# yondonfu/ai-rtc-agent

Hardware: NVIDIA H100
Metric: frames/sec at 512x512 SD-Turbo img2img (1-step, stream-batch 1) (higher is better)
Workload: dtype f16

## Files before the change

### ai-rtc-agent_b200/csrc/epilogue.cuh

```cuda
#pragma once
#include "igemm.cuh"
#include "ptx.cuh"
#include "wgmma.cuh"

namespace b2 {

__device__ __forceinline__ float gelu_erf(float x) {
    return 0.5f * x * (1.0f + erff(x * 0.70710678118654752440f));
}

__device__ __forceinline__ void store_half16(__half* dst, const float* v, int nv, bool vec_ok) {
    if (nv == 16 && vec_ok) {
        uint4 u[2];
        __half2* h = reinterpret_cast<__half2*>(u);
#pragma unroll
        for (int i = 0; i < 8; ++i) h[i] = __floats2half2_rn(v[2 * i], v[2 * i + 1]);
        reinterpret_cast<uint4*>(dst)[0] = u[0];
        reinterpret_cast<uint4*>(dst)[1] = u[1];
    } else {
#pragma unroll
        for (int i = 0; i < 16; ++i)
            if (i < nv) dst[i] = __float2half_rn(v[i]);
    }
}
// ... 97 lines not shown
struct EpiRow {
    long orow;
    int b;
    bool ok;
    float mu, rstd;
};

__device__ __forceinline__ void store_half2(__half* dst, float x0, float x1, bool two, bool vec_ok) {
    if (two && vec_ok) {
        *reinterpret_cast<__half2*>(dst) = __floats2half2_rn(x0, x1);
    } else {
        dst[0] = __float2half_rn(x0);
        if (two) dst[1] = __float2half_rn(x1);
    }
}

__device__ __forceinline__ void rowstat_quad(const IgEpilogue& e, const EpiRow& rw, float s1, float s2, int lane) {
    s1 += __shfl_xor_sync(0xffffffffu, s1, 1);
    s2 += __shfl_xor_sync(0xffffffffu, s2, 1);
    s1 += __shfl_xor_sync(0xffffffffu, s1, 2);
    s2 += __shfl_xor_sync(0xffffffffu, s2, 2);
    if ((lane & 3) == 0 && rw.ok) rowstat_add(e, rw.orow, s1, s2);
}

template <int BN>
__device__ __forceinline__ void epi_frag(const IgEpilogue& e, const float (&acc)[BN / 2], const EpiRow (&rw)[2], int ntile,
                                         bool ln_fma, int lane) {
    const int q2 = 2 * (lane & 3);
    const bool vec_out = (e.ldc & 1) == 0;
    if (e.flags & IG_GEGLU) {
        constexpr int HALF = BN / 2;
        const int pv0 = ntile * BN, oc0 = ntile * HALF;
#pragma unroll
        for (int j = 0; j < HALF / 8; ++j) {
            const int c = 8 * j + q2;
#pragma unroll
            for (int h = 0; h < 2; ++h) {
                if (!rw[h].ok) continue;
                float v[2];
#pragma unroll
                for (int u = 0; u < 2; ++u) {
                    float a = acc[4 * j + 2 * h + u], g = acc[4 * (j + HALF / 8) + 2 * h + u];
                    const int pv = pv0 + c + u, pg = pv0 + HALF + c + u;
                    if (ln_fma) {
                        const float nmr = -rw[h].mu * rw[h].rstd;
                        a = fmaf(rw[h].rstd, a, fmaf(nmr, e.colsum[pv], e.colbias ? e.colbias[pv] : 0.f));
                        g = fmaf(rw[h].rstd, g, fmaf(nmr, e.colsum[pg], e.colbias ? e.colbias[pg] : 0.f));
                    } else {
                        if (e.colsum) {
                            a = rw[h].rstd * (a - rw[h].mu * e.colsum[pv]);
                            g = rw[h].rstd * (g - rw[h].mu * e.colsum[pg]);
                        }
                        if (e.colbias) {
                            a += e.colbias[pv];
                            g += e.colbias[pg];
                        }
                    }
                    v[u] = a * gelu_erf(g);
                }
                store_half2(e.out + rw[h].orow * e.ldc + oc0 + c, v[0], v[1], true, vec_out);
            }
        }
        return;
    }
    float s1[2] = {0.f, 0.f}, s2[2] = {0.f, 0.f};
#pragma unroll
    for (int j = 0; j < BN / 8; ++j) {
        const int col = ntile * BN + 8 * j + q2;
        if (col >= e.n_valid) continue;
        const bool two = col + 1 < e.n_valid;
        const bool transposed = e.out2 && col >= e.col2;
#pragma unroll
        for (int h = 0; h < 2; ++h) {
            if (!rw[h].ok) continue;
            float x[2] = {acc[4 * j + 2 * h], acc[4 * j + 2 * h + 1]};
            const float* bp = e.colbias ? e.colbias + (long)rw[h].b * e.colbias_bstride + col : nullptr;
            if (ln_fma) {
                const float nmr = -rw[h].mu * rw[h].rstd;
#pragma unroll
                for (int u = 0; u < 2; ++u)
                    x[u] = fmaf(rw[h].rstd, x[u], fmaf(nmr, e.colsum[col + u], bp && (u == 0 || two) ? bp[u] : 0.f));
            } else {
                if (e.colsum) {
#pragma unroll
                    for (int u = 0; u < 2; ++u)
                        if (u == 0 || two) x[u] = rw[h].rstd * (x[u] - rw[h].mu * e.colsum[col + u]);
                }
                if (bp) {
                    x[0] += bp[0];
                    if (two) x[1] += bp[1];
                }
                if (e.acc_scale != 1.0f) {
                    x[0] *= e.acc_scale;
                    x[1] *= e.acc_scale;
                }
                if (e.res) {
                    const __half* rp = e.res + rw[h].orow * e.ldr + col;
                    if (two && (e.ldr & 1) == 0) {
                        const float2 f = __half22float2(*reinterpret_cast<const __half2*>(rp));
                        x[0] += e.res_scale * f.x;
                        x[1] += e.res_scale * f.y;
                    } else {
                        x[0] += e.res_scale * __half2float(rp[0]);
                        if (two) x[1] += e.res_scale * __half2float(rp[1]);
                    }
                }
                if (e.flags & IG_RELU) {
                    x[0] = fmaxf(x[0], 0.f);
                    x[1] = fmaxf(x[1], 0.f);
                }
            }
            if (transposed) {
                __half* tp = e.out2 + (long)(col - e.col2) * e.ld2 + rw[h].orow;
                tp[0] = __float2half_rn(x[0]);
                if (two) tp[e.ld2] = __float2half_rn(x[1]);
                continue;
            }
            if (e.rowstat_out && !ln_fma) {
                const float r0 = __half2float(__float2half_rn(x[0]));
                const float r1 = two ? __half2float(__float2half_rn(x[1])) : 0.f;
                s1[h] += r0 + r1;
                s2[h] += r0 * r0 + r1 * r1;
            }
            store_half2(e.out + rw[h].orow * e.ldc + col, x[0], x[1], two, vec_out);
        }
    }
    if (e.rowstat_out && !ln_fma) {
        rowstat_quad(e, rw[0], s1[0], s2[0], lane);
        rowstat_quad(e, rw[1], s1[1], s2[1], lane);
    }
}

template <int BN>
__device__ __forceinline__ void frag_to_smem(float* dst, const float (&acc)[BN / 2], int r0, int lane, int c0, int nc, bool colmajor) {
    const int q2 = 2 * (lane & 3);
#pragma unroll
    for (int j = 0; j < BN / 8; ++j) {
        const int c = 8 * j + q2 - c0;
        if (c < 0 || c >= nc) continue;
#pragma unroll
        for (int h = 0; h < 2; ++h) {
            const int r = r0 + 8 * h;
            if (colmajor) {
                dst[c * 128 + r] = acc[4 * j + 2 * h];
                dst[(c + 1) * 128 + r] = acc[4 * j + 2 * h + 1];
            } else {
                *reinterpret_cast<float2*>(dst + (((c >> 2) * 128 + r) << 2) + (c & 3)) =
                    make_float2(acc[4 * j + 2 * h], acc[4 * j + 2 * h + 1]);
            }
        }
    }
}

}
```

### ai-rtc-agent_b200/csrc/igemm.cu

```cuda
#include "igemm.cuh"

#include <cudaTypedefs.h>
#include <stdarg.h>
#include <stdio.h>
#include <stdlib.h>
#include <string.h>

#include "epilogue.cuh"
#include "launch.cuh"
#include "ptx.cuh"

namespace b2 {

#ifdef B2_TIMELINE
#define B2_TS(stmt) stmt
#else
#define B2_TS(stmt)
#endif

static thread_local char g_err[1024] = "";
const char* b2_last_error() { return g_err; }
void b2_set_error(const char* fmt, ...) {
    va_list ap;
    va_start(ap, fmt);
// ... 114 lines not shown
    const int cr = PAIR ? (int)(blockIdx.x & 1) : 0;
    const int mt_first = (int)blockIdx.x;
    const int mt_step = (int)gridDim.x;
    const int mt_guard = PAIR ? cr : 0;

    const int num_mtiles = p.tiles_w * p.tiles_h * p.tiles_n;
    const int ntile = blockIdx.y;
    const int kb_begin = blockIdx.z * p.kb_per_split;
    const int kb_end = min(p.total_kb, kb_begin + p.kb_per_split);
    [[maybe_unused]] unsigned long long* ts = p.dbg_ts ? p.dbg_ts + ((size_t)(blockIdx.z * gridDim.y + blockIdx.y) * gridDim.x + blockIdx.x) * 8 : nullptr;
    B2_TS(if (ts && threadIdx.x == 0) ts[0] = globaltimer_ns();)

    if (threadIdx.x == IG_CONS) {
        for (int s = 0; s < p.nseg; ++s) tma_prefetch_desc(&p.tmA[s]);
        tma_prefetch_desc(&p.tmB);
        for (int s = 0; s < p.num_stages; ++s) {
            mbar_init(&full_bar[s], 1);
            mbar_init(&empty_bar[s], (PAIR ? 2 : 1) * (IG_CONS / 32));
        }
        fence_mbar_init();
    }
    if (PAIR) {
        cluster_arrive_relaxed();
        cluster_wait();
    }
    __syncthreads();

    pdl_launch_dependents();
    pdl_wait();
    B2_TS(if (ts && threadIdx.x == 0) ts[1] = globaltimer_ns();)

    if (warp == IG_CONS / 32) {
        if (lane == 0) {
            [[maybe_unused]] const uint16_t pair_mask = PAIR ? (uint16_t)(3u << (cluster_ctarank() & ~1u)) : (uint16_t)0;
            int stage = 0;
            uint32_t phase = 0;
            for (int mt = mt_first; mt - mt_guard < num_mtiles; mt += mt_step) {
                const int w0 = (mt % p.tiles_w) * p.tw, h0 = ((mt / p.tiles_w) % p.tiles_h) * p.th;
                const int n0 = (mt / (p.tiles_w * p.tiles_h)) * p.tn;
                int seg = 0, base = 0;
                while (seg < p.nseg - 1 && kb_begin >= base + p.seg_ntap[seg] * p.seg_cblocks[seg]) {
                    base += p.seg_ntap[seg] * p.seg_cblocks[seg];
                    ++seg;
                }
                int tap = (kb_begin - base) / p.seg_cblocks[seg];
                int cb = (kb_begin - base) % p.seg_cblocks[seg];
                for (int kb = kb_begin; kb < kb_end; ++kb) {
                    mbar_wait(&empty_bar[stage], phase ^ 1);
#ifdef B2_BOUND_STUDY
                    if (p.dbg_mode == 1 && kb >= kb_begin + p.num_stages) {
                        mbar_arrive(&full_bar[stage]);
                        if (++stage == p.num_stages) { stage = 0; phase ^= 1; }
                        continue;
                    }
#endif
                    mbar_expect_tx(&full_bar[stage], p.a_bytes + p.b_bytes);
                    uint8_t* sa = smem + (size_t)stage * stage_bytes;
                    uint8_t* sb = sa + A_BYTES;
                    int dy = 0, dx = 0;
                    if (p.seg_ntap[seg] == 9) {
                        dy = tap / 3 - 1;
                        dx = tap % 3 - 1;
                    }
                    tma_load_4d(p.swap ? sb : sa, &p.tmA[seg], &full_bar[stage], p.seg_c0[seg] + cb * IG_BK,
                                w0 * p.stride + dx, h0 * p.stride + dy, n0);
                    if (PAIR)
                        tma_load_2d_mc(sb + cr * (BN / 2) * 128, &p.tmB, &full_bar[stage], kb * IG_BK, ntile * BN + cr * (BN / 2), pair_mask);
                    else
                        tma_load_2d(p.swap ? sa : sb, &p.tmB, &full_bar[stage], kb * IG_BK, ntile * (p.swap ? IG_BM : BN));
                    B2_TS(if (ts && mt == (int)blockIdx.x && kb == kb_begin) ts[2] = globaltimer_ns();)
                    if (++cb == p.seg_cblocks[seg]) {
                        cb = 0;
                        if (++tap == p.seg_ntap[seg]) {
                            tap = 0;
                            ++seg;
                        }
                    }
                    if (++stage == p.num_stages) {
                        stage = 0;
                        phase ^= 1;
                    }
                }
            }
        }
    } else {
        const int wg = warp >> 2;
        const int r0 = wg * 64 + (warp & 3) * 16 + (lane >> 2);
        [[maybe_unused]] const uint32_t peer_empty = PAIR ? dsmem_map(smem_u32(empty_bar), cluster_ctarank() ^ 1u) : 0u;
        const IgEpilogue& e = p.epi;
        const bool ln_fma = e.colsum && !p.swap && !(e.flags & IG_SPLITK) && (e.ldc & 7) == 0 && (e.n_valid & 15) == 0;
        const uint32_t smem_base = smem_u32(smem);
        auto release = [&](int s) {
            if (lane == 0) {
                mbar_arrive(&empty_bar[s]);
                if (PAIR) mbar_arrive_remote(peer_empty + (uint32_t)s * 8u);
            }
        };
        int stage = 0;
        uint32_t phase = 0;
        int it = 0;
        for (int mt = mt_first; mt - mt_guard < num_mtiles; mt += mt_step, ++it) {
            float acc[BN / 2];
#pragma unroll
            for (int i = 0; i < BN / 2; ++i) acc[i] = 0.f;
            int prev = -1;
            for (int kb = kb_begin; kb < kb_end; ++kb) {
                mbar_wait(&full_bar[stage], phase);
                B2_TS(if (ts && it == 0 && kb == kb_begin && threadIdx.x == 0) ts[3] = globaltimer_ns();)
                const uint32_t sa = smem_base + (uint32_t)stage * stage_bytes;
                const uint64_t da = make_kmajor_sw128_desc(sa + (uint32_t)wg * (64 * 128));
                const uint64_t db = make_kmajor_sw128_desc(sa + A_BYTES);
#ifdef B2_BOUND_STUDY
                if (p.dbg_mode != 2)
#endif
                {
                    wgmma_fence_regs(acc);
                    wgmma_fence();
#pragma unroll
                    for (int k = 0; k < 4; ++k) Wgmma<BN>::ss(acc, da + 2 * k, db + 2 * k, 1u);
                    wgmma_commit();
                    wgmma_wait<1>();
                    wgmma_fence_regs(acc);
                }
                if (prev >= 0) release(prev);
                prev = stage;
                if (++stage == p.num_stages) {
                    stage = 0;
                    phase ^= 1;
                }
            }
            wgmma_wait<0>();
            wgmma_fence_regs(acc);
            if (prev >= 0) release(prev);
            B2_TS(if (ts && it == 0 && threadIdx.x == 0) ts[4] = globaltimer_ns();)

            const int w0 = (mt % p.tiles_w) * p.tw, h0 = ((mt / p.tiles_w) % p.tiles_h) * p.th;
            const int n0 = (mt / (p.tiles_w * p.tiles_h)) * p.tn;
            if (p.swap || (e.flags & IG_SPLITK)) {
                float* stg = reinterpret_cast<float*>(smem);
                cons_bar_sync();
                if (e.flags & IG_SPLITK) {
                    frag_to_smem<BN>(stg, acc, r0, lane, 0, BN, false);
                } else {
                    for (int c = 0; c < BN; c += SWAP_CH) {
                        SwapPre pre;
                        swap_prefetch(p, pre, SWAP_CH, c, ntile, n0, h0, w0, threadIdx.x);
                        frag_to_smem<BN>(stg, acc, r0, lane, c, SWAP_CH, true);
                        cons_bar_sync();
                        swap_store_chunk(p, pre, stg, ntile, threadIdx.x);
                        cons_bar_sync();
                    }
                }
            } else {
                EpiRow rw[2];
#pragma unroll
                for (int h = 0; h < 2; ++h) {
                    const int r = r0 + 8 * h;
                    const int wi = r % p.tw, hi = (r / p.tw) % p.th, ni = r / (p.tw * p.th);
                    const int n = n0 + ni, hh = h0 + hi, ww = w0 + wi;
                    rw[h].ok = (ni < p.tn) && (n < p.Nb) && (hh < p.Ho) && (ww < p.Wo);
                    rw[h].orow = ((long)n * p.Ho + hh) * p.Wo + ww;
                    rw[h].b = n;
                    ln_row_stats(e, rw[h].orow, rw[h].ok, rw[h].mu, rw[h].rstd);
                }
                epi_frag<BN>(e, acc, rw, ntile, ln_fma, lane);
            }
            B2_TS(if (ts && it == 0 && threadIdx.x == 0) ts[5] = globaltimer_ns();)
        }
    }
    if (p.epi.flags & IG_SPLITK) {
        const int mt = blockIdx.x;
        const int w0 = (mt % p.tiles_w) * p.tw, h0 = ((mt / p.tiles_w) % p.tiles_h) * p.th;
        const int n0 = (mt / (p.tiles_w * p.tiles_h)) * p.tn;
        const int splits = (int)gridDim.z;
        const int rk_mul = PAIR ? 2 : 1, rk_add = cr;
        cluster_sync_all();
        B2_TS(if (ts && threadIdx.x == 0) ts[6] = globaltimer_ns();)
        if (warp < IG_CONS / 32 && p.swap) {
            const int rank = (int)cluster_ctarank();
            const int cols_per = BN / splits;
            const int ch = cols_per < SWAP_CH ? cols_per : SWAP_CH;
            const int t = threadIdx.x & (IG_BM - 1);
            const int half = threadIdx.x >> 7;
            const uint32_t stg_local = smem_u32(smem);
            float* T = reinterpret_cast<float*>(smem + (size_t)BN * IG_BM * 4);
            for (int c = rank * cols_per; c < (rank + 1) * cols_per; c += ch) {
                SwapPre pre;
                swap_prefetch(p, pre, ch, c, ntile, n0, h0, w0, threadIdx.x);
                if (ch >= 16) {
                    for (int g = 4 * half; g < (ch >> 2); g += 8) {
                        float acc[16];
                        const int cc = ((c >> 2) + g) >> 2;
                        switch (splits) {
                            case 2: splitk_sum16<2>(stg_local, cc, t, acc); break;
                            case 4: splitk_sum16<4>(stg_local, cc, t, acc); break;
                            default: splitk_sum16<8>(stg_local, cc, t, acc); break;
                        }
#pragma unroll
                        for (int i = 0; i < 16; ++i) T[(4 * g + i) * IG_BM + t] = acc[i];
                    }
                } else {
                    const int gg = half;
                    float4 v[8];
#pragma unroll
                    for (int sidx = 0; sidx < 8; ++sidx)
                        v[sidx] = dsmem_ld_f4(dsmem_map(stg_local, (uint32_t)sidx) + (uint32_t)((((c >> 2) + gg) * IG_BM + t) * 16));
                    float4 a = make_float4(0.f, 0.f, 0.f, 0.f);
#pragma unroll
                    for (int sidx = 0; sidx < 8; ++sidx) { a.x += v[sidx].x; a.y += v[sidx].y; a.z += v[sidx].z; a.w += v[sidx].w; }
                    T[(4 * gg + 0) * IG_BM + t] = a.x;
                    T[(4 * gg + 1) * IG_BM + t] = a.y;
                    T[(4 * gg + 2) * IG_BM + t] = a.z;
                    T[(4 * gg + 3) * IG_BM + t] = a.w;
                }
                cons_bar_sync();
                swap_store_chunk(p, pre, T, ntile, threadIdx.x);
                cons_bar_sync();
            }
        } else if (warp < IG_CONS / 32) {
            const int rank = (int)cluster_ctarank() / rk_mul;
            const int rows_per = IG_BM / splits;
            const int t = threadIdx.x;
            const int chunks = BN >> 4;
            const uint32_t stg_local = smem_u32(smem);
            for (int item = t; item < rows_per * chunks; item += IG_CONS) {
                const int rl = item % rows_per;
                const int cc = item / rows_per;
                const int r = rank * rows_per + rl;
                const int wi = r % p.tw, hi = (r / p.tw) % p.th, ni = r / (p.tw * p.th);
                const int n = n0 + ni, h = h0 + hi, w = w0 + wi;
                const bool ok = (ni < p.tn) && (n < p.Nb) && (h < p.Ho) && (w < p.Wo);
                float acc[16];
                switch (splits) {
                    case 2: splitk_sum16<2>(stg_local, cc, r, acc, rk_mul, rk_add); break;
                    case 4: splitk_sum16<4>(stg_local, cc, r, acc, rk_mul, rk_add); break;
                    default: splitk_sum16<8>(stg_local, cc, r, acc, rk_mul, rk_add); break;
                }
                if (ok) {
                    const long orow = ((long)n * p.Ho + h) * p.Wo + w;
                    float mu, rstd;
                    ln_row_stats(p.epi, orow, true, mu, rstd);
                    epi_store16<0>(p.epi, acc, n, orow, ntile * BN + cc * 16, mu, rstd);
                }
            }
        }
        B2_TS(if (ts && threadIdx.x == 0) ts[7] = globaltimer_ns();)
        cluster_sync_all();
    }
    if (PAIR) {
        cluster_arrive_relaxed();
        cluster_wait();
    }
}

template <int BN, bool PAIR>
__global__ void __launch_bounds__(IG_THREADS, 1) igemm_kernel(const __grid_constant__ IgemmParams p) { igemm_body<BN, PAIR>(p); }

using IgemmFn = void (*)(IgemmParams);
template <bool PAIR>
static IgemmFn igemm_fn(int bn) {
    switch (bn) {
#define B2_IG_CASE(N) case N: if constexpr (PAIR && (N % 32)) return nullptr; else return igemm_kernel<N, PAIR>;
        B2_IG_CASE(16) B2_IG_CASE(32) B2_IG_CASE(48) B2_IG_CASE(64) B2_IG_CASE(80) B2_IG_CASE(96) B2_IG_CASE(112) B2_IG_CASE(128)
        B2_IG_CASE(144) B2_IG_CASE(160) B2_IG_CASE(176) B2_IG_CASE(192) B2_IG_CASE(208) B2_IG_CASE(224) B2_IG_CASE(240) B2_IG_CASE(256)
#undef B2_IG_CASE
        default: return nullptr;
    }
}

static PFN_cuTensorMapEncodeTiled_v12000 get_encode() {
    static PFN_cuTensorMapEncodeTiled_v12000 fn = nullptr;
    if (fn) return fn;
    void* p = nullptr;
    cudaDriverEntryPointQueryResult qres;
    cudaError_t err = cudaGetDriverEntryPoint("cuTensorMapEncodeTiled", &p, cudaEnableDefault, &qres);
    if (err != cudaSuccess || qres != cudaDriverEntryPointSuccess || !p) {
        b2_set_error("cudaGetDriverEntryPoint(cuTensorMapEncodeTiled) failed: %s",
                     cudaGetErrorString(err));
        return nullptr;
    }
    fn = reinterpret_cast<PFN_cuTensorMapEncodeTiled_v12000>(p);
    return fn;
}

static thread_local bool g_plan_dry = false;
void igemm_set_dry_run(bool on) { g_plan_dry = on; }

static int encode_act_map(CUtensorMap* m, const ActView& a, int box_c, int box_w, int box_h, int box_n,
                          int estride) {
    if (g_plan_dry) return 0;
    auto enc = get_encode();
    if (!enc) return -1;
    cuuint64_t dims[4] = {(cuuint64_t)a.C, (cuuint64_t)a.W, (cuuint64_t)a.H, (cuuint64_t)a.N};
    cuuint64_t strides[3] = {(cuuint64_t)a.ld * 2, (cuuint64_t)a.W * a.ld * 2,
                             (cuuint64_t)a.H * a.W * a.ld * 2};
    cuuint32_t box[4] = {(cuuint32_t)box_c, (cuuint32_t)box_w, (cuuint32_t)box_h, (cuuint32_t)box_n};
    cuuint32_t es[4] = {1, (cuuint32_t)estride, (cuuint32_t)estride, 1};
    CUresult r = enc(m, CU_TENSOR_MAP_DATA_TYPE_FLOAT16, 4, const_cast<__half*>(a.ptr), dims, strides,
                     box, es, CU_TENSOR_MAP_INTERLEAVE_NONE, CU_TENSOR_MAP_SWIZZLE_128B,
                     CU_TENSOR_MAP_L2_PROMOTION_L2_256B, CU_TENSOR_MAP_FLOAT_OOB_FILL_NONE);
    if (r != CUDA_SUCCESS) {
        b2_set_error("cuTensorMapEncodeTiled(act) failed: %d (ptr %p dims %d,%d,%d,%d ld %d box "
                     "%d,%d,%d,%d es %d)",
                     (int)r, a.ptr, a.C, a.W, a.H, a.N, a.ld, box_c, box_w, box_h, box_n, estride);
        return -1;
    }
    return 0;
}

static int encode_w_map(CUtensorMap* m, const __half* w, int rows, int ld, int box_rows) {
    if (g_plan_dry) return 0;
    auto enc = get_encode();
    if (!enc) return -1;
    cuuint64_t dims[2] = {(cuuint64_t)ld, (cuuint64_t)rows};
    cuuint64_t strides[1] = {(cuuint64_t)ld * 2};
    cuuint32_t box[2] = {IG_BK, (cuuint32_t)box_rows};
    cuuint32_t es[2] = {1, 1};
    CUresult r = enc(m, CU_TENSOR_MAP_DATA_TYPE_FLOAT16, 2, const_cast<__half*>(w), dims, strides, box,
                     es, CU_TENSOR_MAP_INTERLEAVE_NONE, CU_TENSOR_MAP_SWIZZLE_128B,
                     CU_TENSOR_MAP_L2_PROMOTION_L2_256B, CU_TENSOR_MAP_FLOAT_OOB_FILL_NONE);
    if (r != CUDA_SUCCESS) {
        b2_set_error("cuTensorMapEncodeTiled(weights) failed: %d (rows %d ld %d box %d)", (int)r, rows,
                     ld, box_rows);
        return -1;
    }
    return 0;
}

size_t igemm_partial_floats(int splits, long rows_total, int n_valid) {
    long n_pad = ((n_valid + 255) / 256 + 1) * 256;
    return (size_t)splits * rows_total * n_pad;
}

static int plan_swap(const IgemmDesc& d, IgemmPlan* plan) {
    IgemmParams& p = plan->p;
    if ((d.epi.flags & IG_GEGLU) || d.nseg < 1 || d.nseg > IG_MAX_SRC || d.epi.rowstat_out || d.epi.colsum || d.epi.out2) {
        b2_set_error("igemm(swap): unsupported (GEGLU / LayerNorm fold / row statistics / transposed V / nseg %d)", d.nseg);
        return -1;
    }
    int BN = d.BN;
    const long rows_total = (long)d.Nb * d.Ho * d.Wo;
    if (BN <= 0) BN = rows_total >= 256 ? 256 : (rows_total >= 128 ? 128 : 64);
    if (BN != 64 && BN != 128 && BN != 256) {
        b2_set_error("igemm(swap): BN %d must be 64, 128 or 256", BN);
        return -1;
    }
    p.swap = 1;
    { static const char* dm = getenv("B2_DBG_MODE"); p.dbg_mode = dm ? atoi(dm) : 0; }
    p.acc_bufs = 1;
    p.BN = BN;
    auto lg = [](int v) { int l = 0; while ((1 << l) < v) ++l; return l; };
    int tw, th, tn;
    if (d.Ho == 1 && d.Nb == 1) { tw = BN; th = 1; tn = 1; }
    else if (d.Wo >= 16) { tw = 16; th = BN / 16; tn = 1; }
    else { tw = 8; th = 8; tn = BN / 64; }
    p.tw = tw; p.th = th; p.tn = tn;
    p.tw_log2 = lg(tw); p.th_log2 = lg(th);
    p.tiles_w = (d.Wo + tw - 1) / tw;
    p.tiles_h = (d.Ho + th - 1) / th;
    p.tiles_n = (d.Nb + tn - 1) / tn;
    p.Wo = d.Wo; p.Ho = d.Ho; p.Nb = d.Nb;
    p.stride = d.stride < 1 ? 1 : d.stride;
    p.nseg = d.nseg;
    int total_kb = 0;
    for (int s = 0; s < d.nseg; ++s) {
        const ActView& a = d.src[s];
        if (a.C % IG_BK != 0 || (a.ld % 8) != 0 || (reinterpret_cast<uintptr_t>(a.ptr) & 15) || (d.ntap[s] != 1 && d.ntap[s] != 9)) {
            b2_set_error("igemm(swap): bad source %d", s);
            return -1;
        }
        p.seg_ntap[s] = d.ntap[s];
        p.seg_cblocks[s] = a.C / IG_BK;
        p.seg_c0[s] = 0;
        total_kb += d.ntap[s] * p.seg_cblocks[s];
        if (encode_act_map(&p.tmA[s], a, IG_BK, tw * p.stride, th * p.stride, tn, p.stride)) return -1;
    }
    p.total_kb = total_kb;
    if (d.w_ld < total_kb * IG_BK || (d.w_ld % 8) != 0 || (reinterpret_cast<uintptr_t>(d.w) & 15)) {
        b2_set_error("igemm(swap): weight ld %d < K %d or misaligned", d.w_ld, total_kb * IG_BK);
        return -1;
    }
    if (encode_w_map(&p.tmB, d.w, d.w_rows, d.w_ld, IG_BM)) return -1;
    p.a_bytes = IG_BM * IG_BK * 2;
    p.b_bytes = (uint32_t)BN * IG_BK * 2;
    int splits = d.splits < 1 ? 1 : d.splits;
    if (splits > total_kb) splits = total_kb;
    if (splits >= 8) splits = 8; else if (splits >= 4) splits = 4; else if (splits >= 2) splits = 2;
    p.kb_per_split = (total_kb + splits - 1) / splits;
    while (splits > 1 && (total_kb + p.kb_per_split - 1) / p.kb_per_split != splits) {
        splits >>= 1;
        p.kb_per_split = (total_kb + splits - 1) / splits;
    }
    plan->splits = splits;
    plan->rows_total = rows_total;
    p.epi = d.epi;
    p.dbg_ts = d.dbg_ts;
    if (splits > 1) p.epi.flags |= IG_SPLITK;
    const int c_tiles = (d.epi.n_valid + IG_BM - 1) / IG_BM;
    p.n_pad = c_tiles * IG_BM;
    if ((d.epi.n_valid & 7) || (d.epi.ldc & 7) || (d.epi.res && (d.epi.ldr & 7)) || (d.epi.colbias && (d.epi.colbias_bstride & 3)) ||
        (reinterpret_cast<uintptr_t>(d.epi.out) & 15) || (reinterpret_cast<uintptr_t>(d.epi.res) & 15) ||
        (reinterpret_cast<uintptr_t>(d.epi.colbias) & 15)) {
        b2_set_error("igemm(swap): epilogue needs n_valid/ldc/ldr multiples of 8 and 16-byte aligned pointers");
        return -1;
    }
    const size_t stage_bytes = (size_t)IG_BM * IG_BK * 2 + (size_t)BN * IG_BK * 2;
    static const char* sw_stage_env = getenv("B2_SWAP_STAGE_KB");
    int stages = (int)(((size_t)(sw_stage_env ? atoi(sw_stage_env) : (d.ring_kb > 0 ? d.ring_kb : 200)) * 1024) / stage_bytes);
    if (stages < 2) stages = 2;
    if (stages > IG_MAX_STAGES) stages = IG_MAX_STAGES;
    if (stages > p.kb_per_split) stages = p.kb_per_split < 2 ? 2 : p.kb_per_split;
    size_t pipe_bytes = stages * stage_bytes;
    {
        const int cols_per = BN / splits;
        const size_t need = (splits > 1 ? (size_t)BN * IG_BM * 4 : 0) + (size_t)(cols_per < SWAP_CH ? cols_per : SWAP_CH) * IG_BM * 4;
        if (need > pipe_bytes) {
            stages = (int)((need + stage_bytes - 1) / stage_bytes);
            if (stages > IG_MAX_STAGES) {
                b2_set_error("igemm(swap): split-K staging does not fit (BN %d)", BN);
                return -1;
            }
            pipe_bytes = stages * stage_bytes;
        }
    }
    p.num_stages = stages;
    plan->smem = pipe_bytes + 1024 + 512;
    uint32_t cols = 32;
    while (cols < (uint32_t)BN) cols <<= 1;
    p.tmem_cols = cols;
    plan->grid = dim3(p.tiles_w * p.tiles_h * p.tiles_n, c_tiles, splits);
    plan->mode = 0;
    return 0;
}

int b2_device_sms() {
    static int sms = 0;
    if (sms == 0) {
        int dev = 0, n = 0;
        if (cudaGetDevice(&dev) == cudaSuccess && cudaDeviceGetAttribute(&n, cudaDevAttrMultiProcessorCount, dev) == cudaSuccess && n > 0)
            sms = n;
        else
            sms = IG_SMS;
        cudaGetLastError();
    }
    return sms;
}

static int igemm_ctas_per_sm(int bn, bool pair) {
    if (g_plan_dry) return 1;
    IgemmFn fn = pair ? igemm_fn<true>(bn) : igemm_fn<false>(bn);
    int n = 0;
    if (fn && cudaOccupancyMaxActiveBlocksPerMultiprocessor(&n, fn, IG_THREADS, 0) == cudaSuccess && n > 0) return n;
    cudaGetLastError();
    return 1;
}

int igemm_plan(const IgemmDesc& d, IgemmPlan* plan) {
    *plan = IgemmPlan{};
    if (d.swap) return plan_swap(d, plan);
    IgemmParams& p = plan->p;
    if (d.nseg < 1 || d.nseg > IG_MAX_SRC) {
        b2_set_error("igemm: bad nseg %d", d.nseg);
        return -1;
    }
    const bool geglu = (d.epi.flags & IG_GEGLU) != 0;
    const int n_gemm = geglu ? d.epi.n_valid * 2 : d.epi.n_valid;
    int BN = d.BN;
    if (BN <= 0) {
        if (n_gemm <= 256 && n_gemm % 16 == 0) BN = n_gemm;
        else if (n_gemm < 16) BN = 16;
        else if (n_gemm % 128 == 0) BN = 128;
        else if (n_gemm % 160 == 0) BN = 160;
        else if (n_gemm % 64 == 0) BN = 64;
        else BN = 128;
    }
    if (BN % 16 != 0 || BN < 16 || BN > 256 || (geglu && (BN % 32 != 0 || n_gemm % BN != 0))) {
        b2_set_error("igemm: unsupported BN %d (n %d)", BN, n_gemm);
        return -1;
    }
    const bool pair = d.pair != 0;
    if (pair && BN % 32 != 0) {
        b2_set_error("igemm(pair): BN %d must be a multiple of 32", BN);
        return -1;
    }
    p.BN = BN;
    { static const char* dm = getenv("B2_DBG_MODE"); p.dbg_mode = dm ? atoi(dm) : 0; }
    const int n_tiles = (n_gemm + BN - 1) / BN;
    if (d.w_rows < n_gemm) {
        if (d.w_rows <= 0) {
            b2_set_error("igemm: w_rows %d", d.w_rows);
            return -1;
        }
    }
    int tw, th, tn;
    if (d.Ho == 1 && d.Nb == 1) {
        tw = IG_BM; th = 1; tn = 1;
    } else {
        if (d.Wo <= 16) tw = d.Wo;
        else if (d.Wo % 16 == 0) tw = 16;
        else if (d.Wo % 8 == 0) tw = 8;
        else tw = 16;
        th = IG_BM / tw;
        if (th > d.Ho) th = d.Ho;
        tn = IG_BM / (tw * th);
        if (tn > d.Nb) tn = d.Nb;
        if (tn < 1) tn = 1;
    }
    p.tw = tw; p.th = th; p.tn = tn;
    p.tiles_w = (d.Wo + tw - 1) / tw;
    p.tiles_h = (d.Ho + th - 1) / th;
    p.tiles_n = (d.Nb + tn - 1) / tn;
    p.Wo = d.Wo; p.Ho = d.Ho; p.Nb = d.Nb;
    p.stride = d.stride < 1 ? 1 : d.stride;
    if (p.stride > 2) {
        b2_set_error("igemm: stride %d", p.stride);
        return -1;
    }
    p.nseg = d.nseg;
    int total_kb = 0;
    for (int s = 0; s < d.nseg; ++s) {
        const ActView& a = d.src[s];
        if (a.C % IG_BK != 0 || (a.ld % 8) != 0 || (reinterpret_cast<uintptr_t>(a.ptr) & 15)) {
            b2_set_error("igemm: source %d: C=%d must be a multiple of 64, ld=%d multiple of 8, ptr "
                         "16B aligned",
                         s, a.C, a.ld);
            return -1;
        }
        if (d.ntap[s] != 1 && d.ntap[s] != 9) {
            b2_set_error("igemm: ntap %d", d.ntap[s]);
            return -1;
        }
        p.seg_ntap[s] = d.ntap[s];
        p.seg_cblocks[s] = a.C / IG_BK;
        p.seg_c0[s] = 0;
        total_kb += d.ntap[s] * p.seg_cblocks[s];
        if (encode_act_map(&p.tmA[s], a, IG_BK, tw * p.stride, th * p.stride, tn, p.stride)) return -1;
    }
    p.total_kb = total_kb;
    if (d.w_ld < total_kb * IG_BK || (d.w_ld % 8) != 0 || (reinterpret_cast<uintptr_t>(d.w) & 15)) {
        b2_set_error("igemm: weight ld %d < K %d or misaligned", d.w_ld, total_kb * IG_BK);
        return -1;
    }
    const int b_rows = pair ? BN / 2 : BN;
    if (encode_w_map(&p.tmB, d.w, d.w_rows, d.w_ld, b_rows)) return -1;
    p.a_bytes = (uint32_t)(tw * th * tn) * IG_BK * 2;
    p.b_bytes = (uint32_t)BN * IG_BK * 2;
    int splits = d.splits < 1 ? 1 : d.splits;
    if (splits > total_kb) splits = total_kb;
    if (pair && splits > 4) splits = 4;
    if (splits >= 8) splits = 8;
    else if (splits >= 4) splits = 4;
    else if (splits >= 2) splits = 2;
    p.kb_per_split = (total_kb + splits - 1) / splits;
    while (splits > 1 && (total_kb + p.kb_per_split - 1) / p.kb_per_split != splits) {
        splits >>= 1;
        p.kb_per_split = (total_kb + splits - 1) / splits;
    }
    plan->splits = splits;
    plan->rows_total = (long)d.Nb * d.Ho * d.Wo;
    p.epi = d.epi;
    p.dbg_ts = d.dbg_ts;
    p.n_pad = n_tiles * BN;
    if (splits > 1) {
        if (geglu) {
            b2_set_error("igemm: split-K cannot be combined with GEGLU");
            return -1;
        }
        p.epi.flags |= IG_SPLITK;
    }
    const size_t stage_bytes = (size_t)IG_BM * IG_BK * 2 + (size_t)BN * IG_BK * 2;
    const int per_sm = igemm_ctas_per_sm(BN, pair);
    const long resident = (long)per_sm * b2_device_sms();
    static const char* pc_env = getenv("B2_PERSIST_CTAS");
    const long persist_ctas = pc_env ? atoi(pc_env) : resident;
    const long all_tiles = (long)p.tiles_w * p.tiles_h * p.tiles_n * n_tiles;
    static const bool no_persist_e = getenv("B2_NO_PERSIST") != nullptr;
    const bool will_persist = !no_persist_e && splits == 1 && all_tiles > resident && 2 * BN <= 512;
    const long total_ctas = will_persist ? persist_ctas : all_tiles * splits;
    static const char* stage_env = getenv("B2_STAGE_KB");
    const size_t ring_budget = stage_env ? (size_t)atoi(stage_env) * 1024
                                         : (d.ring_kb > 0 ? (size_t)d.ring_kb * 1024
                                                          : (size_t)((per_sm >= 2 && total_ctas > b2_device_sms() ? 100 : 200) * 1024));
    int stages = (int)(ring_budget / stage_bytes);
    if (stages < 2) stages = 2;
    if (stages > IG_MAX_STAGES) stages = IG_MAX_STAGES;
    if (stages > p.kb_per_split) stages = p.kb_per_split < 2 ? 2 : p.kb_per_split;
    p.num_stages = stages;
    size_t pipe_bytes = stages * stage_bytes;
    if (splits > 1) {
        const size_t stg = (size_t)BN * IG_BM * 4;
        if (stg > pipe_bytes) {
            stages = (int)((stg + stage_bytes - 1) / stage_bytes);
            if (stages > IG_MAX_STAGES) {
                b2_set_error("igemm: split-K staging does not fit (BN %d)", BN);
                return -1;
            }
            p.num_stages = stages;
            pipe_bytes = stages * stage_bytes;
        }
    }
    plan->smem = pipe_bytes + 1024  + 512 ;
    const int m_tiles = p.tiles_w * p.tiles_h * p.tiles_n;
    int grid_x = m_tiles;
    p.acc_bufs = 1;
    if (will_persist) {
        grid_x = (int)(persist_ctas / n_tiles);
        if (grid_x < 1) grid_x = 1;
        if (grid_x > m_tiles) grid_x = m_tiles;
        p.acc_bufs = 2;
    }
    if (pair) {
        grid_x = (p.acc_bufs == 2 && grid_x > 2) ? (grid_x & ~1) : ((grid_x + 1) & ~1);
    }
    uint32_t cols = 32;
    while (cols < (uint32_t)(BN * p.acc_bufs)) cols <<= 1;
    p.tmem_cols = cols;
    plan->grid = dim3(grid_x, n_tiles, splits);
    plan->mode = pair ? 1 : 0;
    plan->pair = pair ? 1 : 0;
    return 0;
}

int igemm_encode_act_map(CUtensorMap* m, const ActView& a, int box_c, int box_w, int box_h, int box_n, int estride) {
    return encode_act_map(m, a, box_c, box_w, box_h, box_n, estride);
}
int igemm_encode_w_map(CUtensorMap* m, const __half* w, int rows, int ld, int box_rows) { return encode_w_map(m, w, rows, ld, box_rows); }

int igemm_init() {
    static bool attr_set = false;
    if (!attr_set) {
        for (int bn = 16; bn <= 256; bn += 16) {
            for (int pair = 0; pair < 2; ++pair) {
                IgemmFn fn = pair ? igemm_fn<true>(bn) : igemm_fn<false>(bn);
                if (!fn) continue;
                cudaError_t e = cudaFuncSetAttribute(fn, cudaFuncAttributeMaxDynamicSharedMemorySize, 227 * 1024);
                if (e != cudaSuccess) {
                    b2_set_error("cudaFuncSetAttribute(igemm BN %d%s): %s", bn, pair ? " pair" : "", cudaGetErrorString(e));
                    return -1;
                }
            }
        }
        if (!get_encode()) return -1;
        attr_set = true;
    }
    return 0;
}

int igemm_launch(const IgemmPlan& plan, cudaStream_t stream) {
    if (igemm_init()) return -1;
    const int cz = plan.splits > 1 ? plan.splits : 1;
    IgemmFn fn = plan.pair ? igemm_fn<true>(plan.p.BN) : igemm_fn<false>(plan.p.BN);
    if (!fn) {
        b2_set_error("igemm launch: no kernel for BN %d%s", plan.p.BN, plan.pair ? " (CTA pair)" : "");
        return -1;
    }
    cudaError_t e = plan.pair ? launch_kc(fn, plan.grid, dim3(IG_THREADS), plan.smem, stream, 2, cz, plan.p)
                              : launch_k(fn, plan.grid, dim3(IG_THREADS), plan.smem, stream, cz, plan.p);
    if (e != cudaSuccess) {
        b2_set_error("igemm launch: %s", cudaGetErrorString(e));
        return -1;
    }
    return 0;
}

}
```

### ai-rtc-agent_b200/csrc/igemm.cuh

```cuda
#pragma once
#include <cuda.h>
#include <cuda_fp16.h>
#include <cuda_runtime.h>
#include <stdint.h>

namespace b2 {

constexpr int IG_BM = 128;
constexpr int IG_BK = 64;
constexpr int IG_MAX_SRC = 3;
constexpr int IG_MAX_STAGES = 8;
constexpr int IG_CONS = 256;
constexpr int IG_THREADS = IG_CONS + 32;
constexpr int IG_SMS = 132;

enum : int {
    IG_RELU = 1,
    IG_GEGLU = 2,
    IG_SPLITK = 4,
};

struct IgEpilogue {
    __half* out;
    int ldc;
    const float* colbias;
    int colbias_bstride;
    const __half* res;
    int ldr;
    float acc_scale;
    float res_scale;
    int flags;
    int n_valid;
    unsigned long long* rowstat_out;
    const unsigned long long* rowstat_in;
    const float* colsum;
    float ln_inv_c, ln_eps;
    __half* out2;
    int ld2, col2;
};

constexpr float IG_STAT_SCALE = 1048576.f;

struct IgemmParams {
    CUtensorMap tmA[IG_MAX_SRC];
    CUtensorMap tmB;
    int seg_ntap[IG_MAX_SRC];
    int seg_cblocks[IG_MAX_SRC];
    int seg_c0[IG_MAX_SRC];
    int nseg;
    int total_kb;
    int kb_per_split;
    int tw, th, tn;
    int tiles_w, tiles_h, tiles_n;
    int Wo, Ho, Nb;
    int stride;
    int BN;
    int num_stages;
    int acc_bufs;
    uint32_t a_bytes;
    uint32_t b_bytes;
    uint32_t tmem_cols;
    unsigned long long* dbg_ts;
    int n_pad;
    int swap;
    int tw_log2, th_log2;
    int dbg_mode;
    IgEpilogue epi;
};

struct ActView {
    const __half* ptr;
    int N, H, W, C;
    int ld;
};

struct IgemmDesc {
    ActView src[IG_MAX_SRC];
    int ntap[IG_MAX_SRC];
    int nseg;
    const __half* w;
    int w_rows;
    int w_ld;
    int stride;
    int Nb, Ho, Wo;
    int BN;
    int swap;
    int splits;
    int ring_kb;
    int max_splits;
    int pair_auto;
    int pair_splits;
    int pair;
    unsigned long long* dbg_ts;
    float* partial;
    int* tile_counters;
    IgEpilogue epi;
};

struct IgemmPlan {
    int mode;
    IgemmParams p;
    dim3 grid;
    size_t smem;
    int splits;
    long rows_total;
    int pair;
};

int igemm_plan(const IgemmDesc& d, IgemmPlan* plan);
int igemm_launch(const IgemmPlan& plan, cudaStream_t stream);
void igemm_set_dry_run(bool on);
int igemm_init();
int b2_device_sms();
size_t igemm_partial_floats(int splits, long rows_total, int n_valid);
const char* b2_last_error();
void b2_set_error(const char* fmt, ...);

}

int igemm_autotile(b2::IgemmDesc d, bool allow_swap, b2::IgemmPlan* plan);
```

Before: 162.1.

## Add halo-tile implicit GEMM kernel reusing one activation load across 3x3 taps

Adds a separate implicit-GEMM kernel for stride-1, non-split 3x3 convolutions. For each channel block it loads one (8+2)x(16+2) halo tile of activations by TMA and feeds all nine taps from it through shifted shared-memory descriptors, instead of loading one activation tile per tap. A and B now have separate rings: a smaller A ring of halo slots and a B ring advanced per tap. The aim is to cut activation TMA traffic and shared-memory fill by roughly nine times. The cost is a fixed 8x16 spatial tile, extra planning logic, and reliance on the descriptor offsets into swizzled halo rows being correct.

```diff
diff --git a/ai-rtc-agent_b200/csrc/epilogue.cuh b/ai-rtc-agent_b200/csrc/epilogue.cuh
--- a/ai-rtc-agent_b200/csrc/epilogue.cuh
+++ b/ai-rtc-agent_b200/csrc/epilogue.cuh
@@ -273,4 +273,22 @@
     }
 }
 
-}
+template <int BN>
+__device__ __forceinline__ void epi_tile(const IgemmParams& p, const float (&acc)[BN / 2], int r0, int n0, int h0, int w0, int ntile,
+                                         bool ln_fma, int lane) {
+    const IgEpilogue& e = p.epi;
+    EpiRow rw[2];
+#pragma unroll
+    for (int h = 0; h < 2; ++h) {
+        const int r = r0 + 8 * h;
+        const int wi = r % p.tw, hi = (r / p.tw) % p.th, ni = r / (p.tw * p.th);
+        const int n = n0 + ni, hh = h0 + hi, ww = w0 + wi;
+        rw[h].ok = (ni < p.tn) && (n < p.Nb) && (hh < p.Ho) && (ww < p.Wo);
+        rw[h].orow = ((long)n * p.Ho + hh) * p.Wo + ww;
+        rw[h].b = n;
+        ln_row_stats(e, rw[h].orow, rw[h].ok, rw[h].mu, rw[h].rstd);
+    }
+    epi_frag<BN>(e, acc, rw, ntile, ln_fma, lane);
+}
+
+}
diff --git a/ai-rtc-agent_b200/csrc/igemm.cu b/ai-rtc-agent_b200/csrc/igemm.cu
--- a/ai-rtc-agent_b200/csrc/igemm.cu
+++ b/ai-rtc-agent_b200/csrc/igemm.cu
@@ -290,18 +290,7 @@
                     }
                 }
             } else {
-                EpiRow rw[2];
-#pragma unroll
-                for (int h = 0; h < 2; ++h) {
-                    const int r = r0 + 8 * h;
-                    const int wi = r % p.tw, hi = (r / p.tw) % p.th, ni = r / (p.tw * p.th);
-                    const int n = n0 + ni, hh = h0 + hi, ww = w0 + wi;
-                    rw[h].ok = (ni < p.tn) && (n < p.Nb) && (hh < p.Ho) && (ww < p.Wo);
-                    rw[h].orow = ((long)n * p.Ho + hh) * p.Wo + ww;
-                    rw[h].b = n;
-                    ln_row_stats(e, rw[h].orow, rw[h].ok, rw[h].mu, rw[h].rstd);
-                }
-                epi_frag<BN>(e, acc, rw, ntile, ln_fma, lane);
+                epi_tile<BN>(p, acc, r0, n0, h0, w0, ntile, ln_fma, lane);
             }
             B2_TS(if (ts && it == 0 && threadIdx.x == 0) ts[5] = globaltimer_ns();)
         }
@@ -394,7 +383,6 @@
 template <int BN, bool PAIR>
 __global__ void __launch_bounds__(IG_THREADS, 1) igemm_kernel(const __grid_constant__ IgemmParams p) { igemm_body<BN, PAIR>(p); }
 
-using IgemmFn = void (*)(IgemmParams);
 template <bool PAIR>
 static IgemmFn igemm_fn(int bn) {
     switch (bn) {
@@ -584,9 +572,14 @@
     return sms;
 }
 
-static int igemm_ctas_per_sm(int bn, bool pair) {
+static IgemmFn kernel_for(int bn, bool pair, bool halo) {
+    if (halo) return igemm_halo_fn(bn, pair);
+    return pair ? igemm_fn<true>(bn) : igemm_fn<false>(bn);
+}
+
+static int igemm_ctas_per_sm(int bn, bool pair, bool halo) {
     if (g_plan_dry) return 1;
-    IgemmFn fn = pair ? igemm_fn<true>(bn) : igemm_fn<false>(bn);
+    IgemmFn fn = kernel_for(bn, pair, halo);
     int n = 0;
     if (fn && cudaOccupancyMaxActiveBlocksPerMultiprocessor(&n, fn, IG_THREADS, 0) == cudaSuccess && n > 0) return n;
     cudaGetLastError();
@@ -630,8 +623,19 @@
             return -1;
         }
     }
+    bool halo = d.stride <= 1 && d.splits <= 1 && d.Ho >= IG_HALO_TH;
+    bool has3x3 = false;
+    for (int s = 0; s < d.nseg; ++s) {
+        if (d.ntap[s] != 9) continue;
+        has3x3 = true;
+        halo = halo && d.src[s].H == d.Ho && d.src[s].W == d.Wo && d.src[s].N == d.Nb;
+    }
+    halo = halo && has3x3;
+    p.halo = halo ? 1 : 0;
     int tw, th, tn;
-    if (d.Ho == 1 && d.Nb == 1) {
+    if (halo) {
+        tw = IG_HALO_TW; th = IG_HALO_TH; tn = 1;
+    } else if (d.Ho == 1 && d.Nb == 1) {
         tw = IG_BM; th = 1; tn = 1;
     } else {
         if (d.Wo <= 16) tw = d.Wo;
@@ -672,7 +676,8 @@
         p.seg_cblocks[s] = a.C / IG_BK;
         p.seg_c0[s] = 0;
         total_kb += d.ntap[s] * p.seg_cblocks[s];
-        if (encode_act_map(&p.tmA[s], a, IG_BK, tw * p.stride, th * p.stride, tn, p.stride)) return -1;
+        const int halo_px = halo && d.ntap[s] == 9 ? 2 : 0;
+        if (encode_act_map(&p.tmA[s], a, IG_BK, tw * p.stride + halo_px, th * p.stride + halo_px, tn, p.stride)) return -1;
     }
     p.total_kb = total_kb;
     if (d.w_ld < total_kb * IG_BK || (d.w_ld % 8) != 0 || (reinterpret_cast<uintptr_t>(d.w) & 15)) {
@@ -707,7 +712,7 @@
         p.epi.flags |= IG_SPLITK;
     }
     const size_t stage_bytes = (size_t)IG_BM * IG_BK * 2 + (size_t)BN * IG_BK * 2;
-    const int per_sm = igemm_ctas_per_sm(BN, pair);
+    const int per_sm = igemm_ctas_per_sm(BN, pair, halo);
     const long resident = (long)per_sm * b2_device_sms();
     static const char* pc_env = getenv("B2_PERSIST_CTAS");
     const long persist_ctas = pc_env ? atoi(pc_env) : resident;
@@ -725,6 +730,17 @@
     if (stages > p.kb_per_split) stages = p.kb_per_split < 2 ? 2 : p.kb_per_split;
     p.num_stages = stages;
     size_t pipe_bytes = stages * stage_bytes;
+    if (halo) {
+        const size_t b_ring = (size_t)stages * BN * IG_BK * 2;
+        int a_units = 0;
+        for (int s = 0; s < d.nseg; ++s) a_units += p.seg_cblocks[s];
+        int a_stages = ring_budget > b_ring ? (int)((ring_budget - b_ring) / IG_HALO_SLOT) : 0;
+        if (a_stages > a_units) a_stages = a_units;
+        if (a_stages > IG_MAX_STAGES) a_stages = IG_MAX_STAGES;
+        if (a_stages < 2) a_stages = 2;
+        p.a_stages = a_stages;
+        pipe_bytes = b_ring + (size_t)a_stages * IG_HALO_SLOT;
+    }
     if (splits > 1) {
         const size_t stg = (size_t)BN * IG_BM * 4;
         if (stg > pipe_bytes) {
@@ -768,12 +784,14 @@
     static bool attr_set = false;
     if (!attr_set) {
         for (int bn = 16; bn <= 256; bn += 16) {
-            for (int pair = 0; pair < 2; ++pair) {
-                IgemmFn fn = pair ? igemm_fn<true>(bn) : igemm_fn<false>(bn);
+            for (int k = 0; k < 4; ++k) {
+                const bool pair = k & 1, halo = k & 2;
+                IgemmFn fn = kernel_for(bn, pair, halo);
                 if (!fn) continue;
                 cudaError_t e = cudaFuncSetAttribute(fn, cudaFuncAttributeMaxDynamicSharedMemorySize, 227 * 1024);
                 if (e != cudaSuccess) {
-                    b2_set_error("cudaFuncSetAttribute(igemm BN %d%s): %s", bn, pair ? " pair" : "", cudaGetErrorString(e));
+                    b2_set_error("cudaFuncSetAttribute(igemm%s BN %d%s): %s", halo ? " halo" : "", bn, pair ? " pair" : "",
+                                 cudaGetErrorString(e));
                     return -1;
                 }
             }
@@ -787,9 +805,9 @@
 int igemm_launch(const IgemmPlan& plan, cudaStream_t stream) {
     if (igemm_init()) return -1;
     const int cz = plan.splits > 1 ? plan.splits : 1;
-    IgemmFn fn = plan.pair ? igemm_fn<true>(plan.p.BN) : igemm_fn<false>(plan.p.BN);
+    IgemmFn fn = kernel_for(plan.p.BN, plan.pair, plan.p.halo);
     if (!fn) {
-        b2_set_error("igemm launch: no kernel for BN %d%s", plan.p.BN, plan.pair ? " (CTA pair)" : "");
+        b2_set_error("igemm launch: no %skernel for BN %d%s", plan.p.halo ? "halo " : "", plan.p.BN, plan.pair ? " (CTA pair)" : "");
         return -1;
     }
     cudaError_t e = plan.pair ? launch_kc(fn, plan.grid, dim3(IG_THREADS), plan.smem, stream, 2, cz, plan.p)
diff --git a/ai-rtc-agent_b200/csrc/igemm.cuh b/ai-rtc-agent_b200/csrc/igemm.cuh
--- a/ai-rtc-agent_b200/csrc/igemm.cuh
+++ b/ai-rtc-agent_b200/csrc/igemm.cuh
@@ -13,6 +13,9 @@
 constexpr int IG_CONS = 256;
 constexpr int IG_THREADS = IG_CONS + 32;
 constexpr int IG_SMS = 132;
+constexpr int IG_HALO_TW = 8, IG_HALO_TH = 16;
+constexpr uint32_t IG_HALO_BYTES = (IG_HALO_TW + 2) * (IG_HALO_TH + 2) * IG_BK * 2;
+constexpr uint32_t IG_HALO_SLOT = (IG_HALO_BYTES + 1023u) & ~1023u;
 
 enum : int {
     IG_RELU = 1,
@@ -65,6 +68,8 @@
     int swap;
     int tw_log2, th_log2;
     int dbg_mode;
+    int halo;
+    int a_stages;
     IgEpilogue epi;
 };
 
@@ -107,6 +112,9 @@
     int pair;
 };
 
+using IgemmFn = void (*)(IgemmParams);
+IgemmFn igemm_halo_fn(int bn, bool pair);
+
 int igemm_plan(const IgemmDesc& d, IgemmPlan* plan);
 int igemm_launch(const IgemmPlan& plan, cudaStream_t stream);
 void igemm_set_dry_run(bool on);
diff --git a/ai-rtc-agent_b200/csrc/igemm_halo.cu b/ai-rtc-agent_b200/csrc/igemm_halo.cu
--- /dev/null
+++ b/ai-rtc-agent_b200/csrc/igemm_halo.cu
@@ -0,0 +1,183 @@
+#include "igemm.cuh"
+
+#include "epilogue.cuh"
+#include "launch.cuh"
+#include "ptx.cuh"
+
+namespace b2 {
+
+template <int BN, bool PAIR>
+__device__ __forceinline__ void igemm_body_halo(const IgemmParams& p) {
+    extern __shared__ uint8_t smem_raw[];
+    uint8_t* smem = reinterpret_cast<uint8_t*>((reinterpret_cast<uintptr_t>(smem_raw) + 1023) &
+                                               ~static_cast<uintptr_t>(1023));
+    const int warp = threadIdx.x >> 5;
+    const int lane = threadIdx.x & 31;
+    constexpr uint32_t B_SLOT = (uint32_t)BN * IG_BK * 2;
+    uint8_t* a_ring = smem;
+    uint8_t* b_ring = smem + (size_t)p.a_stages * IG_HALO_SLOT;
+    uint64_t* b_full = reinterpret_cast<uint64_t*>(b_ring + (size_t)p.num_stages * B_SLOT);
+    uint64_t* b_empty = b_full + IG_MAX_STAGES;
+    uint64_t* a_full = b_empty + IG_MAX_STAGES;
+    uint64_t* a_empty = a_full + IG_MAX_STAGES;
+    const int cr = PAIR ? (int)(blockIdx.x & 1) : 0;
+    const int mt_guard = PAIR ? cr : 0;
+    const int num_mtiles = p.tiles_w * p.tiles_h * p.tiles_n;
+    const int ntile = blockIdx.y;
+
+    if (threadIdx.x == IG_CONS) {
+        for (int s = 0; s < p.nseg; ++s) tma_prefetch_desc(&p.tmA[s]);
+        tma_prefetch_desc(&p.tmB);
+        for (int s = 0; s < p.num_stages; ++s) {
+            mbar_init(&b_full[s], 1);
+            mbar_init(&b_empty[s], (PAIR ? 2 : 1) * (IG_CONS / 32));
+        }
+        for (int s = 0; s < p.a_stages; ++s) {
+            mbar_init(&a_full[s], 1);
+            mbar_init(&a_empty[s], IG_CONS / 32);
+        }
+        fence_mbar_init();
+    }
+    if (PAIR) {
+        cluster_arrive_relaxed();
+        cluster_wait();
+    }
+    __syncthreads();
+
+    pdl_launch_dependents();
+    pdl_wait();
+
+    if (warp == IG_CONS / 32) {
+        if (lane == 0) {
+            [[maybe_unused]] const uint16_t pair_mask = PAIR ? (uint16_t)(3u << (cluster_ctarank() & ~1u)) : (uint16_t)0;
+            int bs = 0, as = 0;
+            uint32_t bph = 0, aph = 0;
+            [[maybe_unused]] int a_loads = 0, b_loads = 0;
+            for (int mt = (int)blockIdx.x; mt - mt_guard < num_mtiles; mt += (int)gridDim.x) {
+                const int w0 = (mt % p.tiles_w) * IG_HALO_TW, h0 = ((mt / p.tiles_w) % p.tiles_h) * IG_HALO_TH;
+                const int n0 = mt / (p.tiles_w * p.tiles_h);
+                int kb0 = 0;
+                for (int seg = 0; seg < p.nseg; ++seg) {
+                    const int ntap = p.seg_ntap[seg], ncb = p.seg_cblocks[seg];
+                    const int o = ntap == 9 ? 1 : 0;
+                    for (int cb = 0; cb < ncb; ++cb) {
+                        mbar_wait(&a_empty[as], aph ^ 1);
+#ifdef B2_BOUND_STUDY
+                        if (p.dbg_mode == 1 && a_loads++ >= p.a_stages) mbar_arrive(&a_full[as]);
+                        else
+#endif
+                        {
+                            mbar_expect_tx(&a_full[as], ntap == 9 ? IG_HALO_BYTES : IG_BM * IG_BK * 2);
+                            tma_load_4d(a_ring + (size_t)as * IG_HALO_SLOT, &p.tmA[seg], &a_full[as], p.seg_c0[seg] + cb * IG_BK, w0 - o,
+                                        h0 - o, n0);
+                        }
+                        if (++as == p.a_stages) { as = 0; aph ^= 1; }
+                        for (int tap = 0; tap < ntap; ++tap) {
+                            const int kb = kb0 + tap * ncb + cb;
+                            mbar_wait(&b_empty[bs], bph ^ 1);
+#ifdef B2_BOUND_STUDY
+                            if (p.dbg_mode == 1 && b_loads++ >= p.num_stages) mbar_arrive(&b_full[bs]);
+                            else
+#endif
+                            {
+                                mbar_expect_tx(&b_full[bs], p.b_bytes);
+                                uint8_t* sb = b_ring + (size_t)bs * B_SLOT;
+                                if (PAIR)
+                                    tma_load_2d_mc(sb + cr * (BN / 2) * 128, &p.tmB, &b_full[bs], kb * IG_BK, ntile * BN + cr * (BN / 2), pair_mask);
+                                else
+                                    tma_load_2d(sb, &p.tmB, &b_full[bs], kb * IG_BK, ntile * BN);
+                            }
+                            if (++bs == p.num_stages) { bs = 0; bph ^= 1; }
+                        }
+                    }
+                    kb0 += ntap * ncb;
+                }
+            }
+        }
+    } else {
+        const int wg = warp >> 2;
+        const int r0 = wg * 64 + (warp & 3) * 16 + (lane >> 2);
+        [[maybe_unused]] const uint32_t peer_b_empty = PAIR ? dsmem_map(smem_u32(b_empty), cluster_ctarank() ^ 1u) : 0u;
+        const IgEpilogue& e = p.epi;
+        const bool ln_fma = e.colsum && (e.ldc & 7) == 0 && (e.n_valid & 15) == 0;
+        const uint32_t a_base = smem_u32(a_ring), b_base = smem_u32(b_ring);
+        constexpr int pitch = IG_HALO_TW + 2;
+        int bs = 0, as = 0;
+        uint32_t bph = 0, aph = 0;
+        for (int mt = (int)blockIdx.x; mt - mt_guard < num_mtiles; mt += (int)gridDim.x) {
+            float acc[BN / 2];
+#pragma unroll
+            for (int i = 0; i < BN / 2; ++i) acc[i] = 0.f;
+            int prev_b = -1, prev_a = -1;
+            auto retire = [&]() {
+                if (lane == 0) {
+                    if (prev_b >= 0) {
+                        mbar_arrive(&b_empty[prev_b]);
+                        if (PAIR) mbar_arrive_remote(peer_b_empty + (uint32_t)prev_b * 8u);
+                    }
+                    if (prev_a >= 0) mbar_arrive(&a_empty[prev_a]);
+                }
+                prev_a = -1;
+            };
+            for (int seg = 0; seg < p.nseg; ++seg) {
+                const int ntap = p.seg_ntap[seg], ncb = p.seg_cblocks[seg];
+                for (int cb = 0; cb < ncb; ++cb) {
+                    mbar_wait(&a_full[as], aph);
+                    const uint32_t sa = a_base + (uint32_t)as * IG_HALO_SLOT;
+                    for (int tap = 0; tap < ntap; ++tap) {
+                        mbar_wait(&b_full[bs], bph);
+                        const uint64_t da = ntap == 9 ? make_kmajor_sw128_desc(sa + (uint32_t)((8 * wg + tap / 3) * pitch + tap % 3) * 128u, pitch * 128)
+                                                      : make_kmajor_sw128_desc(sa + (uint32_t)wg * (64 * 128));
+                        const uint64_t db = make_kmajor_sw128_desc(b_base + (uint32_t)bs * B_SLOT);
+#ifdef B2_BOUND_STUDY
+                        if (p.dbg_mode != 2)
+#endif
+                        {
+                            wgmma_fence_regs(acc);
+                            wgmma_fence();
+#pragma unroll
+                            for (int k = 0; k < 4; ++k) Wgmma<BN>::ss(acc, da + 2 * k, db + 2 * k, 1u);
+                            wgmma_commit();
+                            wgmma_wait<1>();
+                            wgmma_fence_regs(acc);
+                        }
+                        retire();
+                        prev_b = bs;
+                        if (++bs == p.num_stages) { bs = 0; bph ^= 1; }
+                    }
+                    prev_a = as;
+                    if (++as == p.a_stages) { as = 0; aph ^= 1; }
+                }
+            }
+            wgmma_wait<0>();
+            wgmma_fence_regs(acc);
+            retire();
+
+            const int w0 = (mt % p.tiles_w) * IG_HALO_TW, h0 = ((mt / p.tiles_w) % p.tiles_h) * IG_HALO_TH;
+            const int n0 = mt / (p.tiles_w * p.tiles_h);
+            epi_tile<BN>(p, acc, r0, n0, h0, w0, ntile, ln_fma, lane);
+        }
+    }
+    if (PAIR) {
+        cluster_arrive_relaxed();
+        cluster_wait();
+    }
+}
+
+template <int BN, bool PAIR>
+__global__ void __launch_bounds__(IG_THREADS, 1) igemm_halo_kernel(const __grid_constant__ IgemmParams p) { igemm_body_halo<BN, PAIR>(p); }
+
+template <bool PAIR>
+static IgemmFn halo_fn(int bn) {
+    switch (bn) {
+#define B2_IG_CASE(N) case N: if constexpr (PAIR && (N % 32)) return nullptr; else return igemm_halo_kernel<N, PAIR>;
+        B2_IG_CASE(16) B2_IG_CASE(32) B2_IG_CASE(48) B2_IG_CASE(64) B2_IG_CASE(80) B2_IG_CASE(96) B2_IG_CASE(112) B2_IG_CASE(128)
+        B2_IG_CASE(144) B2_IG_CASE(160) B2_IG_CASE(176) B2_IG_CASE(192) B2_IG_CASE(208) B2_IG_CASE(224) B2_IG_CASE(240) B2_IG_CASE(256)
+#undef B2_IG_CASE
+        default: return nullptr;
+    }
+}
+
+IgemmFn igemm_halo_fn(int bn, bool pair) { return pair ? halo_fn<true>(bn) : halo_fn<false>(bn); }
+
+}
```

Result: no change. 164.6, median of 6 (+1.6%).
